# NIH-NEI/oct-image-segmentation-models

Measured on AMD Instinct MI355X. Metric: B-scans/sec (train step), 256x512 3-class U-Net, higher is better.
Workload: dtype f32; 1 GPU; configs[1]: train step (fwd+Dice-macro+bwd+allreduce+Adam), per-GPU batch 32, 256x512x1, 3-class, pool_layers=4, start_neurons=8, random-init weights; global_batch=32, parallelism=dp1, allreduce=none

## Files before the change

oct-image-segmentation-models_amd/csrc/common.hpp:

```cpp
#pragma once
#include <hip/hip_runtime.h>
#include <stdint.h>

namespace oct {

constexpr int kTileX = 32;
constexpr int kTileY = 8;
constexpr int kBlock = 256;

enum { BN_A = 0, BN_B = 1, BN_MEAN = 2, BN_RSTD = 3, BN_C1 = 4, BN_C2 = 5, BN_GA = 6, BN_GB = 7, BN_GD = 8, BN_ARRAYS = 9 };

enum { F_U8 = 1, F_AFF = 2, F_TWO = 4, F_UP = 8, F_DROP = 16 };

static __constant__ float c_u8_lut[256];

__host__ __device__ inline uint32_t drop_hash(uint64_t seed, uint64_t step, uint32_t idx) {
    uint64_t x = seed ^ (step * 0x9E3779B97F4A7C15ull) ^ ((uint64_t)idx * 0xD1B54A32D192ED03ull);
    x ^= x >> 33; x *= 0xff51afd7ed558ccdull;
    x ^= x >> 33; x *= 0xc4ceb9fe1a85ec53ull;
    x ^= x >> 33;
    return (uint32_t)(x >> 32);
}

struct DropCfg {
// ... 32 lines not shown
template <int N, bool WT = false>
__device__ inline void block_reduce_store(float (&v)[N], float* red, float* out, int nvalid) {
    wave_reduce_multi<N>(v);
    const int lane = threadIdx.x & 63, wave = threadIdx.x >> 6;
    red[wave * 64 + lane] = v[0];
    __syncthreads();
    if ((int)threadIdx.x < N && (int)threadIdx.x < nvalid) {
        const int l = threadIdx.x * (64 / N);
        const float r = (red[l] + red[64 + l]) + (red[128 + l] + red[192 + l]);
        if constexpr (WT) __hip_atomic_store(out + threadIdx.x, r, __ATOMIC_RELAXED, __HIP_MEMORY_SCOPE_AGENT);
        else out[threadIdx.x] = r;
    }
    __syncthreads();
}

template <int N>
__host__ __device__ inline int chan_of_lane(int lane) {
    int c = 0, n = N, off = 32;
    while (n > 1) { if (lane & off) c += n / 2; n >>= 1; off >>= 1; }
    return c;
}

__device__ inline void column_sums_f64(const float* __restrict__ part, int rows, int C, int c, double* sh, double& s, double& q) {
    s = 0; q = 0;
    const size_t ld = 2 * (size_t)C;
    int i = threadIdx.x;
    for (; i + 7 * kBlock < rows; i += 8 * kBlock) {
        float a[8], b[8];
#pragma unroll
        for (int k = 0; k < 8; ++k) { const float* r = part + (size_t)(i + k * kBlock) * ld + c; a[k] = r[0]; b[k] = r[C]; }
        s += (((double)a[0] + a[1]) + ((double)a[2] + a[3])) + (((double)a[4] + a[5]) + ((double)a[6] + a[7]));
        q += (((double)b[0] + b[1]) + ((double)b[2] + b[3])) + (((double)b[4] + b[5]) + ((double)b[6] + b[7]));
    }
    {
        float a[7], b[7];
#pragma unroll
        for (int k = 0; k < 7; ++k) {
            const int r_ = i + k * kBlock; const bool ok = r_ < rows;
            const float* r = part + (size_t)(ok ? r_ : 0) * ld + c;
            a[k] = ok ? r[0] : 0.f; b[k] = ok ? r[C] : 0.f;
        }
#pragma unroll
        for (int k = 0; k < 7; ++k) { s += a[k]; q += b[k]; }
    }
#pragma unroll
    for (int o = 32; o > 0; o >>= 1) { s += __shfl_xor(s, o, 64); q += __shfl_xor(q, o, 64); }
    const int wave = threadIdx.x >> 6;
    if ((threadIdx.x & 63) == 0) { sh[wave] = s; sh[4 + wave] = q; }
    __syncthreads();
    s = (sh[0] + sh[1]) + (sh[2] + sh[3]); q = (sh[4] + sh[5]) + (sh[6] + sh[7]);
}

__device__ inline float4 ld4(const float* p) { return *reinterpret_cast<const float4*>(p); }
__device__ inline void st4(float* p, const float4& v) { *reinterpret_cast<float4*>(p) = v; }

typedef unsigned short bf16_t;
__device__ inline float bf2f(bf16_t h) { return __uint_as_float(((uint32_t)h) << 16); }
__device__ inline bf16_t f2bf(float f) {
    const uint32_t u = __float_as_uint(f);
    return (bf16_t)((u + 0x7FFFu + ((u >> 16) & 1u)) >> 16);
}
template <typename AT> __device__ inline float4 lda4(const AT* p);
template <> __device__ inline float4 lda4<float>(const float* p) { return *reinterpret_cast<const float4*>(p); }
template <> __device__ inline float4 lda4<bf16_t>(const bf16_t* p) {
    const uint2 u = *reinterpret_cast<const uint2*>(p);
    return make_float4(__uint_as_float(u.x << 16), __uint_as_float(u.x & 0xFFFF0000u),
                       __uint_as_float(u.y << 16), __uint_as_float(u.y & 0xFFFF0000u));
}
template <typename AT> struct Raw4;
template <> struct Raw4<float> { using type = float4; };
template <> struct Raw4<bf16_t> { using type = uint2; };
template <typename AT> __device__ inline typename Raw4<AT>::type ldraw4(const AT* p);
template <> __device__ inline float4 ldraw4<float>(const float* p) { return *reinterpret_cast<const float4*>(p); }
template <> __device__ inline uint2 ldraw4<bf16_t>(const bf16_t* p) { return *reinterpret_cast<const uint2*>(p); }
template <typename AT> __device__ inline typename Raw4<AT>::type raw_zero4();
template <> __device__ inline float4 raw_zero4<float>() { return make_float4(0.f, 0.f, 0.f, 0.f); }
template <> __device__ inline uint2 raw_zero4<bf16_t>() { return make_uint2(0u, 0u); }
__device__ inline float4 widen4(const float4& r) { return r; }
__device__ inline float4 widen4(const uint2& u) {
    return make_float4(__uint_as_float(u.x << 16), __uint_as_float(u.x & 0xFFFF0000u),
                       __uint_as_float(u.y << 16), __uint_as_float(u.y & 0xFFFF0000u));
}
template <typename AT> __device__ inline void sta4(AT* p, const float4& v);
template <> __device__ inline void sta4<float>(float* p, const float4& v) { *reinterpret_cast<float4*>(p) = v; }
typedef __bf16 bf16x2_hw __attribute__((ext_vector_type(2)));
typedef float f32x2_hw __attribute__((ext_vector_type(2)));
template <> __device__ inline void sta4<bf16_t>(bf16_t* p, const float4& v) {
    uint2 u;
    u.x = __builtin_bit_cast(uint32_t, __builtin_convertvector(f32x2_hw{v.x, v.y}, bf16x2_hw));
    u.y = __builtin_bit_cast(uint32_t, __builtin_convertvector(f32x2_hw{v.z, v.w}, bf16x2_hw));
    *reinterpret_cast<uint2*>(p) = u;
}
template <typename AT> __device__ inline float lda1(const AT* p);
template <> __device__ inline float lda1<float>(const float* p) { return *p; }
template <> __device__ inline float lda1<bf16_t>(const bf16_t* p) { return bf2f(*p); }

}
```

oct-image-segmentation-models_amd/csrc/kernels_bwd.hpp:

```cpp
#pragma once
#include "common.hpp"
#include "kernels_fwd.hpp"

namespace oct {

struct PoolBwdArgs {
    const void* gp;
    const void* z;
    const float* bn;
    void* g;
    float* part;
    int H, W, C, tiles_x, tiles, act_bf16;
    FinDesc fin;
};

template <int C_T, typename AT>
__global__ __launch_bounds__(kBlock) void pool_bwd_k(const PoolBwdArgs A) {
    __shared__ float red[256];
    const int Ho = A.H >> 1, Wo = A.W >> 1;
    const int tx = threadIdx.x & (kTileX - 1), ty = threadIdx.x / kTileX;
    const int tile = blockIdx.x;
    const int xo = (tile % A.tiles_x) * kTileX + tx, yo = (tile / A.tiles_x) * kTileY + ty;
    const int b = blockIdx.z, c0 = blockIdx.y * C_T;
    const bool valid = xo < Wo && yo < Ho;
// ... 165 lines not shown
        const uint4 gr = *reinterpret_cast<const uint4*>(g + i * 8), zr = *reinterpret_cast<const uint4*>(z + i * 8);
        const float4 gv[2] = {widen4(make_uint2(gr.x, gr.y)), widen4(make_uint2(gr.z, gr.w))};
        const float4 zv[2] = {widen4(make_uint2(zr.x, zr.y)), widen4(make_uint2(zr.z, zr.w))};
        bf16_t* out = g + i * 8;
#pragma unroll
        for (int hlf = 0; hlf < 2; ++hlf) {
            const int cc = c + 4 * hlf;
            const float4 ga = ld4(bn + BN_GA * C + cc), gb = ld4(bn + BN_GB * C + cc), gd = ld4(bn + BN_GD * C + cc);
            float4 o;
            o.x = bn_bwd_apply1(ga.x, gb.x, gd.x, gv[hlf].x, zv[hlf].x);
            o.y = bn_bwd_apply1(ga.y, gb.y, gd.y, gv[hlf].y, zv[hlf].y);
            o.z = bn_bwd_apply1(ga.z, gb.z, gd.z, gv[hlf].z, zv[hlf].z);
            o.w = bn_bwd_apply1(ga.w, gb.w, gd.w, gv[hlf].w, zv[hlf].w);
            sta4<bf16_t>(out + 4 * hlf, o);
        }
    }
}

struct HeadBwdArgs {
    const void* z; const float* bn;
    const float* w; const float* bias;
    const unsigned char* labels;
    const double* bc;
    void* g;
    float* part;
    float* wpart;
    int HW, nblk, B, macro; float loss_scale; int act_bf16;
    float focal_w, focal_gamma; const float* focal_cw; float inv_count;
    int focal_clip_mod;
    int bce_on; float bce_inner, bce_scale;
    FinDesc fin;
};

template <int C, int CIN, typename AT>
__global__ __launch_bounds__(kBlock) void head_bwd_k(const HeadBwdArgs A) {
    constexpr int NV = CIN * C + C, NG = (NV + 31) / 32;
    constexpr int CP = CIN <= 4 ? 4 : (CIN <= 8 ? 8 : (CIN <= 16 ? 16 : 32));
    __shared__ float red[256];
    const int b = blockIdx.y;
    float s1[CP], s2[CP], wv[NG * 32];
#pragma unroll
    for (int i = 0; i < CP; ++i) { s1[i] = 0.f; s2[i] = 0.f; }
#pragma unroll
    for (int i = 0; i < NG * 32; ++i) wv[i] = 0.f;
    float num[C], den[C];
#pragma unroll
    for (int c = 0; c < C; ++c) {
        const double* k = A.macro ? A.bc + 2 * (b * C + c) : A.bc + 2 * A.B * C;
        num[c] = (float)k[0]; den[c] = (float)k[1];
    }
    const float scale = (1.f - A.focal_w) * (A.macro ? A.loss_scale / (float)(A.B * C) : A.loss_scale);
    const float fscale = A.focal_w * A.loss_scale * A.inv_count;

    const AT* const zbase = reinterpret_cast<const AT*>(A.z) + (size_t)b * A.HW * CIN;
    auto pix_of = [&](int chunk) { const int px = chunk * kBlock + threadIdx.x; return px < A.HW ? px : 0; };
    float zn[CIN];
    int labn = 0;
    if ((int)blockIdx.x * kBlock < A.HW) {
        const int q = pix_of(blockIdx.x);
        head_load<CIN, AT>(zbase + (size_t)q * CIN, zn);
        labn = A.labels[(size_t)b * A.HW + q];
    }
    for (int chunk = blockIdx.x; chunk * kBlock < A.HW; chunk += gridDim.x) {
        const int px = chunk * kBlock + threadIdx.x;
        const bool valid = px < A.HW;
        const size_t pix = (size_t)b * A.HW + (valid ? px : 0);
        float y[CIN], zr[CIN], p[C];
#pragma unroll
        for (int i = 0; i < CIN; ++i) zr[i] = zn[i];
        const int lab = labn;
        if ((chunk + (int)gridDim.x) * kBlock < A.HW) {
            const int q = pix_of(chunk + gridDim.x);
            head_load<CIN, AT>(zbase + (size_t)q * CIN, zn);
            labn = A.labels[(size_t)b * A.HW + q];
        }
        head_logits<C, CIN>(A.bn, A.w, A.bias, y, zr, p);
        float dp[C], dot = 0.f;
#pragma unroll
        for (int c = 0; c < C; ++c) {
            const float yv = lab == c ? 1.f : 0.f;
            dp[c] = -scale * (2.f * yv * den[c] - num[c]) / (den[c] * den[c]);
            if (fscale != 0.f && lab == c) {
                const bool inr = p[c] >= kFocalEps && p[c] <= 1.f - kFocalEps;
                if (inr || !A.focal_clip_mod) {
                    const float pc = fminf(fmaxf(p[c], kFocalEps), 1.f - kFocalEps);
                    const float q = 1.f - p[c], cw = A.focal_cw ? A.focal_cw[c] : 1.f, qg1 = powf(q, A.focal_gamma - 1.f);
                    dp[c] += fscale * cw * (A.focal_gamma * qg1 * logf(pc) - (inr ? qg1 * q / pc : 0.f));
                }
            }
            dot = fmaf(p[c], dp[c], dot);
        }
        float dlb[C];
#pragma unroll
        for (int c = 0; c < C; ++c) dlb[c] = 0.f;
        if (A.bce_on) {
            float q[C], db[C];
            softmax_complement<C>(p, q);
#pragma unroll
            for (int c = 0; c < C; ++c) {
                const bool inr = valid && p[c] >= kFocalEps && q[c] >= kFocalEps;
                const float r = A.bce_scale / ((lab == c ? p[c] : q[c]) + A.bce_inner);
                db[c] = inr ? (lab == c ? -r : r) : 0.f;
            }
#pragma unroll
            for (int c = 0; c < C; ++c) {
                float o = 0.f;
#pragma unroll
                for (int k = 0; k < C; ++k) if (k != c) o = fmaf(p[k], db[k], o);
                dlb[c] = p[c] * (q[c] * db[c] - o);
            }
        }
        float dl[C];
#pragma unroll
        for (int c = 0; c < C; ++c) { dl[c] = (valid ? p[c] * (dp[c] - dot) : 0.f) + dlb[c]; wv[CIN * C + c] += dl[c]; }
        float g[CIN];
#pragma unroll
        for (int i = 0; i < CIN; ++i) {
            float a = 0.f;
#pragma unroll
            for (int c = 0; c < C; ++c) { a = fmaf(A.w[i * C + c], dl[c], a); wv[i * C + c] = fmaf(y[i], dl[c], wv[i * C + c]); }
            a = (valid && y[i] > 0.f) ? a : 0.f;
            const float xh = (zr[i] - A.bn[BN_MEAN * CIN + i]) * A.bn[BN_RSTD * CIN + i];
            g[i] = a; s1[i] += a; s2[i] += a * xh;
        }
        if (valid) {
#pragma unroll
            for (int i = 0; i < CIN; i += 4) sta4<AT>(reinterpret_cast<AT*>(A.g) + pix * CIN + i, make_float4(g[i], g[i + 1], g[i + 2], g[i + 3]));
        }
    }
    const size_t row = (size_t)b * gridDim.x + blockIdx.x;
    float* out = A.part + row * (2 * CIN);
    block_reduce_store<CP, true>(s1, red, out, CIN);
    block_reduce_store<CP, true>(s2, red, out + CIN, CIN);
    float* wout = A.wpart + row * NV;
#pragma unroll
    for (int gi = 0; gi < NG; ++gi) {
        float t[32];
#pragma unroll
        for (int k = 0; k < 32; ++k) t[k] = wv[gi * 32 + k];
        block_reduce_store<32>(t, red, wout + gi * 32, NV - gi * 32 < 32 ? NV - gi * 32 : 32);
    }
    if (A.fin.counter) {
        __shared__ __attribute__((aligned(16))) char fin_lds[16 + kBlock * 16 + 2 * CP * 8];
        finalize_in_launch(A.fin, A.part, gridDim.x * gridDim.y, CIN, gridDim.x * gridDim.y, fin_lds);
    }
}

struct ConvBwdWArgs {
    const void* x0; const float* ab0; int C0;
    const void* x1; const float* ab1; int C1;
    int flags;
    const void* dz;
    const void* zf; const float* bnf;
    float* part;
    int B, H, W, Cin, Cout, tiles_x, tiles, total_tiles, npb;
    DropCfg drop;
    int act_bf16;
};

__device__ __forceinline__ float fetch_x(const ConvBwdWArgs& A, int b, int iy, int ix, int c) {
    const bool up = (A.flags & F_UP) != 0;
    const int Hs = up ? A.H >> 1 : A.H, Ws = up ? A.W >> 1 : A.W;
    const int sy = up ? iy >> 1 : iy, sx = up ? ix >> 1 : ix;
    const size_t pix = ((size_t)b * Hs + sy) * Ws + sx;
    if (A.flags & F_U8) return c_u8_lut[reinterpret_cast<const unsigned char*>(A.x0)[pix * A.C0 + c]];
    const float* src = reinterpret_cast<const float*>(A.x0); const float* ab = A.ab0; int C = A.C0, cc = c;
    if ((A.flags & F_TWO) && c >= A.C0) { src = reinterpret_cast<const float*>(A.x1); ab = A.ab1; C = A.C1; cc = c - A.C0; }
    float v = src[pix * C + cc];
    if (A.flags & F_AFF) v = fmaxf(fmaf(ab[cc], v, ab[C + cc]), 0.f);
    if (A.flags & F_DROP) v *= drop_mul(A.drop, (uint32_t)(pix * C + cc));
    return v;
}

template <int KH, int CI_T, int CO_T, typename AT>
__global__ __launch_bounds__(kBlock) void conv_bwd_w_k(const ConvBwdWArgs A) {
// ... 8 lines not shown
    float acc[TAPS], accb = 0.f;
#pragma unroll
    for (int k = 0; k < TAPS; ++k) acc[k] = 0.f;

    for (int tl = blockIdx.x; tl < A.total_tiles; tl += A.npb) {
        const int b = tl / A.tiles, tile = tl % A.tiles;
        const int x0 = (tile % A.tiles_x) * kTileX, y0 = (tile / A.tiles_x) * kTileY;
        __syncthreads();
        for (int i = t; i < XH * XW * CI_T; i += kBlock) {
            const int c = i % CI_T, r = i / CI_T, cx = r % XW, cy = r / XW;
            const int iy = y0 + cy - PT, ix = x0 + cx - PT;
            float v = 0.f;
            if (iy >= 0 && iy < A.H && ix >= 0 && ix < A.W && ci0 + c < A.Cin) v = fetch_x(A, b, iy, ix, ci0 + c);
            Xs[i] = v;
        }
        for (int i = t; i < kTileY * kTileX * CO_T; i += kBlock) {
            const int c = i % CO_T, r = i / CO_T, cx = r % kTileX, cy = r / kTileX;
            const int oy = y0 + cy, ox = x0 + cx;
            float v = 0.f;
            if (oy < A.H && ox < A.W && co0 + c < A.Cout) v = lda1<AT>(reinterpret_cast<const AT*>(A.dz) + (((size_t)b * A.H + oy) * A.W + ox) * A.Cout + co0 + c);
            Ds[i] = v;
        }
        __syncthreads();
        for (int p = ps; p < kTileY * kTileX; p += PS) {
            const int py = p / kTileX, pxx = p % kTileX;
            const float d = Ds[p * CO_T + co];
            accb += d;
#pragma unroll
            for (int ky = 0; ky < KH; ++ky)
#pragma unroll
                for (int kx = 0; kx < KW; ++kx)
                    acc[ky * KW + kx] = fmaf(Xs[((py + ky) * XW + pxx + kx) * CI_T + ci], d, acc[ky * KW + kx]);
        }
    }
#pragma unroll
    for (int k = 0; k < TAPS; ++k) Rs[t * (TAPS + 1) + k] = acc[k];
    Rs[t * (TAPS + 1) + TAPS] = accb;
    __syncthreads();
    if (t < NT) {
        const size_t wsize = (size_t)TAPS * A.Cin * A.Cout;
        float* out = A.part + (size_t)blockIdx.x * (wsize + A.Cout);
        const bool ok = (ci0 + ci < A.Cin) && (co0 + co < A.Cout);
        for (int k = 0; k <= TAPS; ++k) {
            float s = 0.f;
            for (int q = 0; q < PS; ++q) s += Rs[(q * NT + t) * (TAPS + 1) + k];
            if (!ok) continue;
            if (k < TAPS) out[((size_t)k * A.Cin + ci0 + ci) * A.Cout + co0 + co] = s;
            else if (ci0 + ci == 0) out[wsize + co0 + co] = s;
        }
    }
}

template <typename AT, bool FUSE>
__global__ __launch_bounds__(kBlock) void conv_dw_first_k(const ConvBwdWArgs A, int tiles_x, int tiles, int total_tiles) {
    constexpr int TH = 8, TW = 128, XH = TH + 2, XW = TW + 2;
    __shared__ float Xs[XH * XW];
    __shared__ float red[256];
    __shared__ float lut_s[256];
    const int t = threadIdx.x, xl = t & 31, row = t >> 5;
    lut_s[t] = c_u8_lut[t];
    float acc0[64], acc1[16];
#pragma unroll
    for (int k = 0; k < 64; ++k) acc0[k] = 0.f;
#pragma unroll
    for (int k = 0; k < 16; ++k) acc1[k] = 0.f;
    const bool u8 = (A.flags & F_U8) != 0;
    for (int tl = blockIdx.x; tl < total_tiles; tl += gridDim.x) {
        const int b = tl / tiles, tile = tl % tiles;
        const int x0 = (tile % tiles_x) * TW, y0 = (tile / tiles_x) * TH;
        __syncthreads();
        {
            constexpr int NS = (XH * XW + kBlock - 1) / kBlock;
            unsigned int rb[NS]; float rf[NS]; bool in[NS];
#pragma unroll
            for (int k = 0; k < NS; ++k) {
                const int i = t + k * kBlock, cy = i / XW, cx = i % XW, iy = y0 + cy - 1, ix = x0 + cx - 1;
                in[k] = i < XH * XW && iy >= 0 && iy < A.H && ix >= 0 && ix < A.W;
                const size_t pix = in[k] ? ((size_t)b * A.H + iy) * A.W + ix : 0;
                rb[k] = 0; rf[k] = 0.f;
                if (in[k]) { if (u8) rb[k] = reinterpret_cast<const unsigned char*>(A.x0)[pix]; else rf[k] = reinterpret_cast<const float*>(A.x0)[pix]; }
            }
#pragma unroll
            for (int k = 0; k < NS; ++k) {
                const int i = t + k * kBlock;
                if (i < XH * XW) Xs[i] = in[k] ? (u8 ? lut_s[rb[k]] : rf[k]) : 0.f;
            }
        }
        __syncthreads();
        const int y = y0 + row;
#pragma unroll
        for (int k = 0; k < TW / 32; ++k) {
            const int xx = xl + 32 * k, x = x0 + xx;
            if (y < A.H && x < A.W) {
                const size_t e8 = (((size_t)b * A.H + y) * A.W + x) * 8;
                const AT* dp = reinterpret_cast<const AT*>(A.dz) + e8;
                const float4 d0 = lda4<AT>(dp), d1 = lda4<AT>(dp + 4);
                float d[8] = {d0.x, d0.y, d0.z, d0.w, d1.x, d1.y, d1.z, d1.w};
                if constexpr (FUSE) {
                    const AT* zp = reinterpret_cast<const AT*>(A.zf) + e8;
                    const float4 z0 = lda4<AT>(zp), z1 = lda4<AT>(zp + 4);
                    const float zv[8] = {z0.x, z0.y, z0.z, z0.w, z1.x, z1.y, z1.z, z1.w};
#pragma unroll
                    for (int co = 0; co < 8; ++co) {
                        const float o = bn_bwd_apply1(A.bnf[BN_GA * 8 + co], A.bnf[BN_GB * 8 + co], A.bnf[BN_GD * 8 + co], d[co], zv[co]);
                        d[co] = dz_as_stored<AT>(o);
                        asm volatile("" : "+v"(d[co]));
                    }
                }
#pragma unroll
                for (int tap = 0; tap < 9; ++tap) {
                    const float xv = Xs[(row + tap / 3) * XW + xx + tap % 3];
#pragma unroll
                    for (int co = 0; co < 8; ++co) {
                        if (tap < 8) acc0[tap * 8 + co] = fmaf(xv, d[co], acc0[tap * 8 + co]);
                        else acc1[co] = fmaf(xv, d[co], acc1[co]);
                    }
                }
#pragma unroll
                for (int co = 0; co < 8; ++co) acc1[8 + co] += d[co];
            }
        }
    }
    float* out = A.part + (size_t)blockIdx.x * 80;
    block_reduce_store<64>(acc0, red, out, 64);
    block_reduce_store<16>(acc1, red, out + 64, 16);
}

template <int JW>
__global__ __launch_bounds__(kBlock) void reduce_partials_k(const float* __restrict__ part, int npb, size_t stride,
                                                           size_t wsize, float* __restrict__ dw, float* __restrict__ db) {
    constexpr int NQ = kBlock / JW;
    __shared__ double sh[NQ][JW];
    const int col = threadIdx.x % JW, q = threadIdx.x / JW;
    const size_t j = (size_t)blockIdx.x * JW + col;
    double s = 0;
    if (j < stride)
        for (int p = q; p < npb; p += NQ) s += part[(size_t)p * stride + j];
    sh[q][col] = s;
    __syncthreads();
    if (q == 0 && j < stride) {
        double t = 0;
#pragma unroll
        for (int k = 0; k < NQ; ++k) t += sh[k][col];
        if (j < wsize) dw[j] = (float)t; else db[j - wsize] = (float)t;
    }
}

struct ReduceAllArgs {
    static constexpr int MAXL = 40;
    int n;
    struct Entry { const float* part; float* dw; float* db; int npb, jw; unsigned stride, wsize, blk_start; } L[MAXL];
};

static __global__ __launch_bounds__(kBlock) void reduce_all_k(const ReduceAllArgs A) {
    __shared__ double sh[kBlock];
    int d = 0;
    while (d + 1 < A.n && blockIdx.x >= A.L[d + 1].blk_start) ++d;
    const ReduceAllArgs::Entry E = A.L[d];
    const int jw = E.jw, nq = kBlock / jw, col = threadIdx.x % jw, q = threadIdx.x / jw;
    const size_t j = (size_t)(blockIdx.x - E.blk_start) * jw + col;
    double s = 0;
    if (j < E.stride) {
        const float* __restrict__ src = E.part + j;
        int p = q;
        for (; p + 7 * nq < E.npb; p += 8 * nq) {
            float v[8];
#pragma unroll
            for (int k = 0; k < 8; ++k) v[k] = src[(size_t)(p + k * nq) * E.stride];
            s += (((double)v[0] + v[1]) + ((double)v[2] + v[3])) + (((double)v[4] + v[5]) + ((double)v[6] + v[7]));
        }
        for (; p < E.npb; p += nq) s += src[(size_t)p * E.stride];
    }
    sh[q * jw + col] = s;
    __syncthreads();
// ... 28 lines not shown
```

oct-image-segmentation-models_amd/csrc/kernels_fwd.hpp:

```cpp
#pragma once
#include "common.hpp"
#include "kernels_fin.hpp"

namespace oct {

struct ConvFwdArgs {
    const void* x0;
    const float* ab0;
    int C0;
    const float* x1;
    const float* ab1;
    int C1;
    const float* w;
    const float* bias;
    void* z;
    float* part;
    int H, W, Cin, Cout, tiles_x, tiles;
    DropCfg drop;
    int act_bf16;
    FinDesc fin;
};

template <int CO_T, int FLAGS>
__device__ inline void accum_src(const void* __restrict__ src, const float* __restrict__ ab, int C, size_t pix,
// ... 36 lines not shown
            if constexpr (U8) v = c_u8_lut[reinterpret_cast<const unsigned char*>(src)[pix * C + c]];
            else v = reinterpret_cast<const float*>(src)[pix * C + c];
            if constexpr (AFF) v = fmaxf(fmaf(ab[c], v, ab[C + c]), 0.f);
        }
        const float* wr = wk + (size_t)c * Cout;
#pragma unroll
        for (int j = 0; j < CO_T; ++j) acc[j] = fmaf(v, wr[j], acc[j]);
    }
}

template <int KH, int CO_T, int FLAGS, typename AT>
__global__ __launch_bounds__(kBlock) void conv_fwd_k(const ConvFwdArgs A) {
    constexpr int KW = KH, PT = (KH - 1) / 2;
    constexpr bool TWO = (FLAGS & F_TWO) != 0, UP = (FLAGS & F_UP) != 0;
    __shared__ float red[256];
    const int tx = threadIdx.x & (kTileX - 1), ty = threadIdx.x / kTileX;
    const int tile = blockIdx.x;
    const int x = (tile % A.tiles_x) * kTileX + tx, y = (tile / A.tiles_x) * kTileY + ty;
    const int b = blockIdx.z, co0 = blockIdx.y * CO_T;
    const bool valid = x < A.W && y < A.H;
    const int Hs = UP ? A.H >> 1 : A.H, Ws = UP ? A.W >> 1 : A.W;

    float acc[CO_T];
#pragma unroll
    for (int j = 0; j < CO_T; ++j) acc[j] = A.bias[co0 + j];

    for (int ky = 0; ky < KH; ++ky) {
        for (int kx = 0; kx < KW; ++kx) {
            const int iy = y + ky - PT, ix = x + kx - PT;
            const bool inb = valid && iy >= 0 && iy < A.H && ix >= 0 && ix < A.W;
            const int sy = UP ? iy >> 1 : iy, sx = UP ? ix >> 1 : ix;
            const size_t pix = inb ? ((size_t)b * Hs + sy) * Ws + sx : 0;
            const float* wk = A.w + (size_t)((ky * KW + kx) * A.Cin) * A.Cout + co0;
            accum_src<CO_T, FLAGS>(A.x0, A.ab0, A.C0, pix, inb, wk, A.Cout, A.drop, acc);
            if constexpr (TWO)
                accum_src<CO_T, FLAGS>(A.x1, A.ab1, A.C1, pix, inb, wk + (size_t)A.C0 * A.Cout, A.Cout, A.drop, acc);
        }
    }
    if (valid) {
        AT* zp = reinterpret_cast<AT*>(A.z) + (((size_t)b * A.H + y) * A.W + x) * A.Cout + co0;
#pragma unroll
        for (int j = 0; j < CO_T; j += 4) sta4<AT>(zp + j, make_float4(acc[j], acc[j + 1], acc[j + 2], acc[j + 3]));
    }
    if (A.part) {
        float s[CO_T], q[CO_T];
#pragma unroll
        for (int j = 0; j < CO_T; ++j) { s[j] = valid ? acc[j] : 0.f; q[j] = s[j] * s[j]; }
        float* out = A.part + ((size_t)b * A.tiles + tile) * (2 * A.Cout);
        block_reduce_store<CO_T>(s, red, out + co0, CO_T);
        block_reduce_store<CO_T>(q, red, out + A.Cout + co0, CO_T);
    }
}

template <typename AT>
__global__ __launch_bounds__(kBlock) void conv_first_fwd_k(const ConvFwdArgs A, int x_is_u8, int tiles_x, int tiles, int total_tiles,
                                                          const float* __restrict__ wgt, const float* __restrict__ bias) {
    constexpr int TH = 8, TW = 128, XH = TH + 2, XW = TW + 2;
    __shared__ float Xs[XH * XW];
    __shared__ float red[256];
    __shared__ float lut_s[256];
    const int t = threadIdx.x, xl = t & 31, row = t >> 5;
    lut_s[t] = c_u8_lut[t];
    float s1[8], s2[8];
#pragma unroll
    for (int j = 0; j < 8; ++j) { s1[j] = 0.f; s2[j] = 0.f; }
    for (int tl = blockIdx.x; tl < total_tiles; tl += gridDim.x) {
        const int b = tl / tiles, tile = tl % tiles;
        const int x0 = (tile % tiles_x) * TW, y0 = (tile / tiles_x) * TH;
        __syncthreads();
        {
            constexpr int NS = (XH * XW + kBlock - 1) / kBlock;
            unsigned int rb[NS]; float rf[NS]; bool in[NS];
#pragma unroll
            for (int k = 0; k < NS; ++k) {
                const int i = t + k * kBlock, cy = i / XW, cx = i % XW, iy = y0 + cy - 1, ix = x0 + cx - 1;
                in[k] = i < XH * XW && iy >= 0 && iy < A.H && ix >= 0 && ix < A.W;
                const size_t pix = in[k] ? ((size_t)b * A.H + iy) * A.W + ix : 0;
                rb[k] = 0; rf[k] = 0.f;
                if (in[k]) { if (x_is_u8) rb[k] = reinterpret_cast<const unsigned char*>(A.x0)[pix]; else rf[k] = reinterpret_cast<const float*>(A.x0)[pix]; }
            }
#pragma unroll
            for (int k = 0; k < NS; ++k) {
                const int i = t + k * kBlock;
                if (i < XH * XW) Xs[i] = in[k] ? (x_is_u8 ? lut_s[rb[k]] : rf[k]) : 0.f;
            }
        }
        __syncthreads();
        const int y = y0 + row;
#pragma unroll
        for (int k = 0; k < TW / 32; ++k) {
            const int xx = xl + 32 * k, x = x0 + xx;
            float acc[8];
#pragma unroll
            for (int j = 0; j < 8; ++j) acc[j] = bias[j];
#pragma unroll
            for (int tap = 0; tap < 9; ++tap) {
                const float xv = Xs[(row + tap / 3) * XW + xx + tap % 3];
#pragma unroll
                for (int j = 0; j < 8; ++j) acc[j] = fmaf(xv, wgt[tap * 8 + j], acc[j]);
            }
            if (y < A.H && x < A.W) {
                AT* zp = reinterpret_cast<AT*>(A.z) + (((size_t)b * A.H + y) * A.W + x) * 8;
                sta4<AT>(zp, make_float4(acc[0], acc[1], acc[2], acc[3]));
                sta4<AT>(zp + 4, make_float4(acc[4], acc[5], acc[6], acc[7]));
#pragma unroll
                for (int j = 0; j < 8; ++j) { s1[j] += acc[j]; s2[j] = fmaf(acc[j], acc[j], s2[j]); }
// ... 64 lines not shown
        const int c = (int)(i % C4) * 4;
        size_t r = i / C4;
        const int xo = (int)(r % Wo); r /= Wo;
        const int yo = (int)(r % Ho); const int b = (int)(r / Ho);
        const float4 a = ld4(ab + c), bb = ld4(ab + C + c);
        float4 m = make_float4(0.f, 0.f, 0.f, 0.f);
#pragma unroll
        for (int dy = 0; dy < 2; ++dy)
#pragma unroll
            for (int dx = 0; dx < 2; ++dx) {
                const float4 v = lda4<AT>(z + (((size_t)b * H + 2 * yo + dy) * W + 2 * xo + dx) * C + c);
                m.x = fmaxf(m.x, fmaf(a.x, v.x, bb.x)); m.y = fmaxf(m.y, fmaf(a.y, v.y, bb.y));
                m.z = fmaxf(m.z, fmaf(a.z, v.z, bb.z)); m.w = fmaxf(m.w, fmaf(a.w, v.w, bb.w));
            }
        sta4<AT>(p + (((size_t)b * Ho + yo) * Wo + xo) * C + c, m);
    }
}

constexpr int kDiceVals = 5;
template <int C> struct DiceN { static constexpr int value = (5 * C <= 16) ? 16 : (5 * C <= 32 ? 32 : 64); };

struct HeadFwdArgs {
    const void* z; const float* ab;
    const float* w; const float* bias;
    float* probs; unsigned char* argmax; const unsigned char* labels;
    float* dice_part;
    int HW, nblk, act_bf16;
    int focal_on; float focal_gamma; const float* focal_cw;
    int focal_clip_mod;
    int bce_on; float bce_inner;
};
constexpr float kFocalEps = 1e-7f;

template <int C>
__device__ inline void softmax_complement(const float (&p)[C], float (&q)[C]) {
#pragma unroll
    for (int c = 0; c < C; ++c) {
        float s = 0.f;
#pragma unroll
        for (int k = 0; k < C; ++k) if (k != c) s += p[k];
        q[c] = s;
    }
}

template <int CIN, typename AT>
__device__ inline void head_load(const AT* __restrict__ zp, float (&zr)[CIN]) {
#pragma unroll
    for (int i = 0; i < CIN; i += 4) {
        const float4 v = lda4<AT>(zp + i);
        zr[i] = v.x; zr[i + 1] = v.y; zr[i + 2] = v.z; zr[i + 3] = v.w;
    }
}

template <int C, int CIN>
__device__ inline void head_logits(const float* __restrict__ ab, const float* __restrict__ w, const float* __restrict__ bias,
                                   float (&y)[CIN], const float (&zr)[CIN], float (&p)[C]) {
#pragma unroll
    for (int i = 0; i < CIN; ++i) y[i] = fmaxf(fmaf(ab[i], zr[i], ab[CIN + i]), 0.f);
    float mx = -3.4e38f;
#pragma unroll
    for (int c = 0; c < C; ++c) {
        float l = bias[c];
#pragma unroll
        for (int i = 0; i < CIN; ++i) l = fmaf(y[i], w[i * C + c], l);
        p[c] = l; mx = fmaxf(mx, l);
    }
    float sum = 0.f;
#pragma unroll
    for (int c = 0; c < C; ++c) { p[c] = expf(p[c] - mx); sum += p[c]; }
    const float inv = 1.f / sum;
#pragma unroll
    for (int c = 0; c < C; ++c) p[c] *= inv;
}

template <int C, int CIN, typename AT>
__global__ __launch_bounds__(kBlock) void head_fwd_k(const HeadFwdArgs A) {
    constexpr int N = DiceN<C>::value;
    __shared__ float red[256];
    const int b = blockIdx.y;
    float v[N];
#pragma unroll
    for (int i = 0; i < N; ++i) v[i] = 0.f;
    for (int chunk = blockIdx.x; chunk * kBlock < A.HW; chunk += gridDim.x) {
        const int px = chunk * kBlock + threadIdx.x;
        const bool valid = px < A.HW;
        const size_t pix = (size_t)b * A.HW + (valid ? px : 0);
        float y[CIN], zr[CIN], p[C];
        head_load<CIN, AT>(reinterpret_cast<const AT*>(A.z) + pix * CIN, zr);
        head_logits<C, CIN>(A.ab, A.w, A.bias, y, zr, p);
        if (valid) {
            if (A.probs) {
#pragma unroll
                for (int c = 0; c < C; ++c) A.probs[pix * C + c] = p[c];
            }
            if (A.argmax) {
                int am = 0; float best = p[0];
#pragma unroll
                for (int c = 1; c < C; ++c) if (p[c] > best) { best = p[c]; am = c; }
                A.argmax[pix] = (unsigned char)am;
            }
            if (A.labels) {
                const int lab = A.labels[pix];
#pragma unroll
                for (int c = 0; c < C; ++c) {
                    const float yv = lab == c ? 1.f : 0.f, ph = p[c] > 0.5f ? 1.f : 0.f;
                    v[c * kDiceVals + 0] += yv * p[c]; v[c * kDiceVals + 1] += yv; v[c * kDiceVals + 2] += p[c];
                    v[c * kDiceVals + 3] += yv * ph;   v[c * kDiceVals + 4] += ph;
                }
                if (A.focal_on) {
                    float py = p[0];
#pragma unroll
                    for (int c = 1; c < C; ++c) py = lab == c ? p[c] : py;
                    const float pc = fminf(fmaxf(py, kFocalEps), 1.f - kFocalEps);
                    const float cw = A.focal_cw ? A.focal_cw[lab < C ? lab : 0] : 1.f;
                    v[C * kDiceVals] += cw * powf(1.f - (A.focal_clip_mod ? pc : py), A.focal_gamma) * -logf(pc);
                }
                if (A.bce_on) {
                    float q[C], t = 0.f;
                    softmax_complement<C>(p, q);
#pragma unroll
                    for (int c = 0; c < C; ++c) {
                        const float u = lab == c ? p[c] : q[c];
                        t -= logf(fminf(fmaxf(u, kFocalEps), 1.f - kFocalEps) + A.bce_inner);
                    }
                    v[C * kDiceVals] += t;
                }
            }
        }
    }
    if (A.labels) block_reduce_store<N>(v, red, A.dice_part + ((size_t)b * gridDim.x + blockIdx.x) * N, N);
}

struct DiceFinArgs {
    const float* part; int B, C, nblk, N;
    float smooth; float* out4; float* out4_user; double* bc;
    int n_user;
    double inv_count;
    float focal_w;
    int bce_on;
};

static __global__ __launch_bounds__(kBlock) void dice_finalize_k(const DiceFinArgs A) {
    __shared__ double sh[8][kBlock];
    double acc[8] = {0, 0, 0, 0, 0, 0, 0, 0};
    const int n = A.B * A.C;
    for (int i = threadIdx.x; i < n; i += kBlock) {
        const int b = i / A.C, c = i % A.C;
        double v[kDiceVals] = {0, 0, 0, 0, 0};
        const float* p0 = A.part + (size_t)b * A.nblk * A.N + c * kDiceVals;
        int k = 0;
        for (; k + 8 <= A.nblk; k += 8) {
            float t[8][kDiceVals];
#pragma unroll
            for (int r = 0; r < 8; ++r)
#pragma unroll
                for (int j = 0; j < kDiceVals; ++j) t[r][j] = p0[(size_t)(k + r) * A.N + j];
#pragma unroll
            for (int r = 0; r < 8; ++r)
#pragma unroll
                for (int j = 0; j < kDiceVals; ++j) v[j] += t[r][j];
        }
        for (; k < A.nblk; ++k)
            for (int j = 0; j < kDiceVals; ++j) v[j] += p0[(size_t)k * A.N + j];
        const double s = A.smooth;
        const double num = 2.0 * v[0] + s, den = v[1] + v[2] + s;
        A.bc[2 * i] = num; A.bc[2 * i + 1] = den;
        acc[0] += num / den;
        acc[1] += (2.0 * v[3] + 1e-5) / (v[1] + v[4] + 1e-5);
        acc[2] += v[0]; acc[3] += v[1]; acc[4] += v[2]; acc[5] += v[3]; acc[6] += v[4];
        if (c == 0)
            for (int k = 0; k < A.nblk; ++k) acc[7] += A.part[((size_t)b * A.nblk + k) * A.N + A.C * kDiceVals];
    }
    for (int j = 0; j < 8; ++j) sh[j][threadIdx.x] = acc[j];
    __syncthreads();
    for (int o = kBlock / 2; o > 0; o >>= 1) {
        if ((int)threadIdx.x < o) for (int j = 0; j < 8; ++j) sh[j][threadIdx.x] += sh[j][threadIdx.x + o];
        __syncthreads();
    }
    if (threadIdx.x == 0) {
        const double s = A.smooth;
        const double num = 2.0 * sh[2][0] + s, den = sh[3][0] + sh[4][0] + s;
        A.bc[2 * n] = num; A.bc[2 * n + 1] = den;
        float o4[8];
        o4[0] = (float)(1.0 - sh[0][0] / n);
        o4[1] = (float)(1.0 - num / den);
        o4[2] = (float)(sh[1][0] / n);
        o4[3] = (float)(2.0 * sh[5][0] / (sh[3][0] + sh[6][0]));
        const double focal = sh[7][0] * A.inv_count, w = A.focal_w;
        o4[4] = (float)focal;
        o4[5] = (float)(w * focal + (1.0 - w) * (1.0 - sh[0][0] / n));
        o4[6] = (float)(w * focal + (1.0 - w) * (1.0 - num / den));
        o4[7] = 0.f;
        if (A.bce_on) {
            const double bce = sh[7][0] * (A.inv_count / A.C);
            o4[4] = (float)bce; o4[5] = 0.f; o4[6] = (float)(bce + (1.0 - num / den));
        }
        for (int j = 0; j < 8; ++j) { A.out4[j] = o4[j]; if (A.out4_user && j < A.n_user) A.out4_user[j] = o4[j]; }
    }
}

static __global__ __launch_bounds__(kBlock) void boundary_maps_k(const unsigned char* __restrict__ lab, unsigned char* __restrict__ out,
                                                         int B, int H, int W, int C, int bg_ilm, int bg_csi) {
    const size_t n = (size_t)B * H * W;
    for (size_t i = (size_t)blockIdx.x * kBlock + threadIdx.x; i < n; i += (size_t)gridDim.x * kBlock) {
        const int c = (int)(i % W); size_t t = i / W;
        const int r = (int)(t % H), b = (int)(t / H);
        const unsigned char* col = lab + (size_t)b * H * W + c;
        auto L = [&](int rr) { return (int)col[(size_t)rr * W]; };
        const int r1 = r + 1 == H ? 0 : r + 1;
        int lv[6];
        const int rows[6] = {r > 0 ? r - 1 : 0, r, r + 1 < H ? r + 1 : H - 1, r1 > 0 ? r1 - 1 : 0, r1, r1 + 1 < H ? r1 + 1 : H - 1};
#pragma unroll
        for (int k = 0; k < 6; ++k) lv[k] = L(rows[k]);
        for (int m = 1; m < C; ++m) {
            const bool flip = (m == 1 && bg_ilm) || (m == C - 1 && bg_csi);
            const int k = flip ? m - 1 : m;
            auto grad2 = [&](int rr, int lo, int mid, int hi) {
                int d2;
                if (H == 1) d2 = 0;
                else if (rr == 0) d2 = 2 * ((hi == k) - (mid == k));
                else if (rr == H - 1) d2 = 2 * ((mid == k) - (lo == k));
                else d2 = (hi == k) - (lo == k);
                if (flip) d2 = -d2;
                return d2 > 0 ? d2 : 0;
            };
            const int g0 = grad2(r, lv[0], lv[1], lv[2]);
// ... 14 lines not shown
```

Measured before the change: 8456 B-scans/s.

## Prefetch head and first-conv tiles, use constant-space loads, parallelize dice finalize

Adds a HeadQueue prefetcher to the forward and backward head kernels so the next chunk's activations and labels load while the current chunk is computed. conv_dw_first_k gets a double-buffered shared input tile with register staging, prefetches dz/zf loads two groups ahead, and raises occupancy via launch_bounds. Small parameter loads now go through the constant address space so they can use scalar loads. dice_finalize uses a deeper unrolled reduction and gives the focal-term sums to otherwise idle threads. These changes aim to hide memory latency, at the cost of more registers and shared memory.

```diff
diff --git a/oct-image-segmentation-models_amd/csrc/common.hpp b/oct-image-segmentation-models_amd/csrc/common.hpp
--- a/oct-image-segmentation-models_amd/csrc/common.hpp
+++ b/oct-image-segmentation-models_amd/csrc/common.hpp
@@ -108,6 +108,7 @@
 }
 
 __device__ inline float4 ld4(const float* p) { return *reinterpret_cast<const float4*>(p); }
+__device__ __forceinline__ float ldc(const float* p) { return *(const __attribute__((address_space(4))) float*)p; }
 __device__ inline void st4(float* p, const float4& v) { *reinterpret_cast<float4*>(p) = v; }
 
 typedef unsigned short bf16_t;
diff --git a/oct-image-segmentation-models_amd/csrc/kernels_bwd.hpp b/oct-image-segmentation-models_amd/csrc/kernels_bwd.hpp
--- a/oct-image-segmentation-models_amd/csrc/kernels_bwd.hpp
+++ b/oct-image-segmentation-models_amd/csrc/kernels_bwd.hpp
@@ -241,28 +241,14 @@
     const float scale = (1.f - A.focal_w) * (A.macro ? A.loss_scale / (float)(A.B * C) : A.loss_scale);
     const float fscale = A.focal_w * A.loss_scale * A.inv_count;
 
-    const AT* const zbase = reinterpret_cast<const AT*>(A.z) + (size_t)b * A.HW * CIN;
-    auto pix_of = [&](int chunk) { const int px = chunk * kBlock + threadIdx.x; return px < A.HW ? px : 0; };
-    float zn[CIN];
-    int labn = 0;
-    if ((int)blockIdx.x * kBlock < A.HW) {
-        const int q = pix_of(blockIdx.x);
-        head_load<CIN, AT>(zbase + (size_t)q * CIN, zn);
-        labn = A.labels[(size_t)b * A.HW + q];
-    }
+    HeadQueue<CIN, kHeadBwdAhead, AT> hq(reinterpret_cast<const AT*>(A.z) + (size_t)b * A.HW * CIN, A.labels + (size_t)b * A.HW, A.HW);
+    hq.fill(blockIdx.x, gridDim.x);
     for (int chunk = blockIdx.x; chunk * kBlock < A.HW; chunk += gridDim.x) {
         const int px = chunk * kBlock + threadIdx.x;
         const bool valid = px < A.HW;
         const size_t pix = (size_t)b * A.HW + (valid ? px : 0);
         float y[CIN], zr[CIN], p[C];
-#pragma unroll
-        for (int i = 0; i < CIN; ++i) zr[i] = zn[i];
-        const int lab = labn;
-        if ((chunk + (int)gridDim.x) * kBlock < A.HW) {
-            const int q = pix_of(chunk + gridDim.x);
-            head_load<CIN, AT>(zbase + (size_t)q * CIN, zn);
-            labn = A.labels[(size_t)b * A.HW + q];
-        }
+        const int lab = hq.pop(zr, chunk + kHeadBwdAhead * (int)gridDim.x);
         head_logits<C, CIN>(A.bn, A.w, A.bias, y, zr, p);
         float dp[C], dot = 0.f;
 #pragma unroll
@@ -273,7 +259,7 @@
                 const bool inr = p[c] >= kFocalEps && p[c] <= 1.f - kFocalEps;
                 if (inr || !A.focal_clip_mod) {
                     const float pc = fminf(fmaxf(p[c], kFocalEps), 1.f - kFocalEps);
-                    const float q = 1.f - p[c], cw = A.focal_cw ? A.focal_cw[c] : 1.f, qg1 = powf(q, A.focal_gamma - 1.f);
+                    const float q = 1.f - p[c], cw = A.focal_cw ? ldc(A.focal_cw + c) : 1.f, qg1 = powf(q, A.focal_gamma - 1.f);
                     dp[c] += fscale * cw * (A.focal_gamma * qg1 * logf(pc) - (inr ? qg1 * q / pc : 0.f));
                 }
             }
@@ -307,9 +293,9 @@
         for (int i = 0; i < CIN; ++i) {
             float a = 0.f;
 #pragma unroll
-            for (int c = 0; c < C; ++c) { a = fmaf(A.w[i * C + c], dl[c], a); wv[i * C + c] = fmaf(y[i], dl[c], wv[i * C + c]); }
+            for (int c = 0; c < C; ++c) { a = fmaf(ldc(A.w + i * C + c), dl[c], a); wv[i * C + c] = fmaf(y[i], dl[c], wv[i * C + c]); }
             a = (valid && y[i] > 0.f) ? a : 0.f;
-            const float xh = (zr[i] - A.bn[BN_MEAN * CIN + i]) * A.bn[BN_RSTD * CIN + i];
+            const float xh = (zr[i] - ldc(A.bn + BN_MEAN * CIN + i)) * ldc(A.bn + BN_RSTD * CIN + i);
             g[i] = a; s1[i] += a; s2[i] += a * xh;
         }
         if (valid) {
@@ -424,9 +410,9 @@
 }
 
 template <typename AT, bool FUSE>
-__global__ __launch_bounds__(kBlock) void conv_dw_first_k(const ConvBwdWArgs A, int tiles_x, int tiles, int total_tiles) {
-    constexpr int TH = 8, TW = 128, XH = TH + 2, XW = TW + 2;
-    __shared__ float Xs[XH * XW];
+__global__ __launch_bounds__(kBlock, 3) void conv_dw_first_k(const ConvBwdWArgs A, int tiles_x, int tiles, int total_tiles) {
+    constexpr int TH = FirstTileRaw::TH, TW = FirstTileRaw::TW, XH = FirstTileRaw::XH, XW = FirstTileRaw::XW, NG = TW / 32;
+    __shared__ float Xs2[2][XH * XW];
     __shared__ float red[256];
     __shared__ float lut_s[256];
     const int t = threadIdx.x, xl = t & 31, row = t >> 5;
@@ -437,44 +423,47 @@
 #pragma unroll
     for (int k = 0; k < 16; ++k) acc1[k] = 0.f;
     const bool u8 = (A.flags & F_U8) != 0;
-    for (int tl = blockIdx.x; tl < total_tiles; tl += gridDim.x) {
+    FirstTileRaw nx;
+    const bool any = (int)blockIdx.x < total_tiles;
+    if (any) nx.request(A.x0, u8, blockIdx.x, tiles, tiles_x, A.H, A.W);
+    __syncthreads();
+    if (any) nx.store(Xs2[0], lut_s, u8);
+    __syncthreads();
+    int cur = 0;
+    for (int tl = blockIdx.x; tl < total_tiles; tl += gridDim.x, cur ^= 1) {
         const int b = tl / tiles, tile = tl % tiles;
         const int x0 = (tile % tiles_x) * TW, y0 = (tile / tiles_x) * TH;
-        __syncthreads();
-        {
-            constexpr int NS = (XH * XW + kBlock - 1) / kBlock;
-            unsigned int rb[NS]; float rf[NS]; bool in[NS];
-#pragma unroll
-            for (int k = 0; k < NS; ++k) {
-                const int i = t + k * kBlock, cy = i / XW, cx = i % XW, iy = y0 + cy - 1, ix = x0 + cx - 1;
-                in[k] = i < XH * XW && iy >= 0 && iy < A.H && ix >= 0 && ix < A.W;
-                const size_t pix = in[k] ? ((size_t)b * A.H + iy) * A.W + ix : 0;
-                rb[k] = 0; rf[k] = 0.f;
-                if (in[k]) { if (u8) rb[k] = reinterpret_cast<const unsigned char*>(A.x0)[pix]; else rf[k] = reinterpret_cast<const float*>(A.x0)[pix]; }
-            }
-#pragma unroll
-            for (int k = 0; k < NS; ++k) {
-                const int i = t + k * kBlock;
-                if (i < XH * XW) Xs[i] = in[k] ? (u8 ? lut_s[rb[k]] : rf[k]) : 0.f;
-            }
-        }
-        __syncthreads();
+        const float* __restrict__ Xs = Xs2[cur];
+        const bool more = tl + (int)gridDim.x < total_tiles;
+        if (more) nx.request(A.x0, u8, tl + gridDim.x, tiles, tiles_x, A.H, A.W);
         const int y = y0 + row;
-#pragma unroll
-        for (int k = 0; k < TW / 32; ++k) {
-            const int xx = xl + 32 * k, x = x0 + xx;
-            if (y < A.H && x < A.W) {
-                const size_t e8 = (((size_t)b * A.H + y) * A.W + x) * 8;
-                const AT* dp = reinterpret_cast<const AT*>(A.dz) + e8;
-                const float4 d0 = lda4<AT>(dp), d1 = lda4<AT>(dp + 4);
-                float d[8] = {d0.x, d0.y, d0.z, d0.w, d1.x, d1.y, d1.z, d1.w};
+        constexpr int AH = 2;
+        float4 dq[NG][2]; [[maybe_unused]] float4 zq[NG][2];
+        bool ok[NG];
+        auto request = [&](int k) {
+            const int x = x0 + xl + 32 * k;
+            ok[k] = y < A.H && x < A.W;
+            const size_t e8 = ok[k] ? (((size_t)b * A.H + y) * A.W + x) * 8 : 0;
+            const AT* dp = reinterpret_cast<const AT*>(A.dz) + e8;
+            dq[k][0] = lda4<AT>(dp); dq[k][1] = lda4<AT>(dp + 4);
+            if constexpr (FUSE) {
+                const AT* zp = reinterpret_cast<const AT*>(A.zf) + e8;
+                zq[k][0] = lda4<AT>(zp); zq[k][1] = lda4<AT>(zp + 4);
+            }
+        };
+#pragma unroll
+        for (int k = 0; k < AH; ++k) request(k);
+#pragma unroll
+        for (int k = 0; k < NG; ++k) {
+            if (k + AH < NG) request(k + AH);
+            const int xx = xl + 32 * k;
+            if (ok[k]) {
+                float d[8] = {dq[k][0].x, dq[k][0].y, dq[k][0].z, dq[k][0].w, dq[k][1].x, dq[k][1].y, dq[k][1].z, dq[k][1].w};
                 if constexpr (FUSE) {
-                    const AT* zp = reinterpret_cast<const AT*>(A.zf) + e8;
-                    const float4 z0 = lda4<AT>(zp), z1 = lda4<AT>(zp + 4);
-                    const float zv[8] = {z0.x, z0.y, z0.z, z0.w, z1.x, z1.y, z1.z, z1.w};
+                    const float zv[8] = {zq[k][0].x, zq[k][0].y, zq[k][0].z, zq[k][0].w, zq[k][1].x, zq[k][1].y, zq[k][1].z, zq[k][1].w};
 #pragma unroll
                     for (int co = 0; co < 8; ++co) {
-                        const float o = bn_bwd_apply1(A.bnf[BN_GA * 8 + co], A.bnf[BN_GB * 8 + co], A.bnf[BN_GD * 8 + co], d[co], zv[co]);
+                        const float o = bn_bwd_apply1(ldc(A.bnf + BN_GA * 8 + co), ldc(A.bnf + BN_GB * 8 + co), ldc(A.bnf + BN_GD * 8 + co), d[co], zv[co]);
                         d[co] = dz_as_stored<AT>(o);
                         asm volatile("" : "+v"(d[co]));
                     }
@@ -492,6 +481,8 @@
                 for (int co = 0; co < 8; ++co) acc1[8 + co] += d[co];
             }
         }
+        if (more) nx.store(Xs2[cur ^ 1], lut_s, u8);
+        __syncthreads();
     }
     float* out = A.part + (size_t)blockIdx.x * 80;
     block_reduce_store<64>(acc0, red, out, 64);
diff --git a/oct-image-segmentation-models_amd/csrc/kernels_fwd.hpp b/oct-image-segmentation-models_amd/csrc/kernels_fwd.hpp
--- a/oct-image-segmentation-models_amd/csrc/kernels_fwd.hpp
+++ b/oct-image-segmentation-models_amd/csrc/kernels_fwd.hpp
@@ -112,6 +112,34 @@
     }
 }
 
+struct FirstTileRaw {
+    static constexpr int TH = 8, TW = 128, XH = TH + 2, XW = TW + 2, NS = (XH * XW + kBlock - 1) / kBlock;
+    unsigned int raw[NS];
+    unsigned int inm;
+    __device__ __forceinline__ void request(const void* __restrict__ x, bool u8, int tl, int tiles, int tiles_x, int H, int W) {
+        const int b = tl / tiles, tile = tl % tiles, x0 = (tile % tiles_x) * TW, y0 = (tile / tiles_x) * TH;
+        inm = 0;
+#pragma unroll
+        for (int k = 0; k < NS; ++k) {
+            const int i = (int)threadIdx.x + k * kBlock, cy = i / XW, cx = i % XW, iy = y0 + cy - 1, ix = x0 + cx - 1;
+            const bool in = i < XH * XW && iy >= 0 && iy < H && ix >= 0 && ix < W;
+            const size_t pix = in ? ((size_t)b * H + iy) * W + ix : 0;
+            raw[k] = 0;
+            if (in) {
+                if (u8) raw[k] = reinterpret_cast<const unsigned char*>(x)[pix]; else raw[k] = __float_as_uint(reinterpret_cast<const float*>(x)[pix]);
+                inm |= 1u << k;
+            }
+        }
+    }
+    __device__ __forceinline__ void store(float* __restrict__ Xs, const float* __restrict__ lut_s, bool u8) const {
+#pragma unroll
+        for (int k = 0; k < NS; ++k) {
+            const int i = (int)threadIdx.x + k * kBlock;
+            if (i < XH * XW) Xs[i] = (inm >> k & 1u) ? (u8 ? lut_s[raw[k]] : __uint_as_float(raw[k])) : 0.f;
+        }
+    }
+};
+
 template <typename AT>
 __global__ __launch_bounds__(kBlock) void conv_first_fwd_k(const ConvFwdArgs A, int x_is_u8, int tiles_x, int tiles, int total_tiles,
                                                           const float* __restrict__ wgt, const float* __restrict__ bias) {
@@ -282,17 +310,49 @@
     }
 }
 
+constexpr int kHeadFwdAhead = 1, kHeadBwdAhead = 1;
+template <int CIN, int D, typename AT>
+struct HeadQueue {
+    const AT* zb; const unsigned char* lb; int HW;
+    float zq[D][CIN]; int lq[D];
+    __device__ HeadQueue(const AT* z, const unsigned char* l, int hw) : zb(z), lb(l), HW(hw) {}
+    __device__ __forceinline__ void request(int d, int chunk) {
+        if (chunk * kBlock < HW) {
+            const int px = chunk * kBlock + (int)threadIdx.x, q = px < HW ? px : 0;
+            head_load<CIN, AT>(zb + (size_t)q * CIN, zq[d]);
+            if (lb) lq[d] = lb[q];
+        }
+    }
+    __device__ __forceinline__ void fill(int first, int stride) {
+#pragma unroll
+        for (int d = 0; d < D; ++d) { lq[d] = 0; request(d, first + d * stride); }
+    }
+    __device__ __forceinline__ int pop(float (&zr)[CIN], int next) {
+        const int lab = lq[0];
+#pragma unroll
+        for (int i = 0; i < CIN; ++i) zr[i] = zq[0][i];
+#pragma unroll
+        for (int d = 0; d + 1 < D; ++d) {
+            lq[d] = lq[d + 1];
+#pragma unroll
+            for (int i = 0; i < CIN; ++i) zq[d][i] = zq[d + 1][i];
+        }
+        request(D - 1, next);
+        return lab;
+    }
+};
+
 template <int C, int CIN>
 __device__ inline void head_logits(const float* __restrict__ ab, const float* __restrict__ w, const float* __restrict__ bias,
                                    float (&y)[CIN], const float (&zr)[CIN], float (&p)[C]) {
 #pragma unroll
-    for (int i = 0; i < CIN; ++i) y[i] = fmaxf(fmaf(ab[i], zr[i], ab[CIN + i]), 0.f);
+    for (int i = 0; i < CIN; ++i) y[i] = fmaxf(fmaf(ldc(ab + i), zr[i], ldc(ab + CIN + i)), 0.f);
     float mx = -3.4e38f;
 #pragma unroll
     for (int c = 0; c < C; ++c) {
-        float l = bias[c];
-#pragma unroll
-        for (int i = 0; i < CIN; ++i) l = fmaf(y[i], w[i * C + c], l);
+        float l = ldc(bias + c);
+#pragma unroll
+        for (int i = 0; i < CIN; ++i) l = fmaf(y[i], ldc(w + i * C + c), l);
         p[c] = l; mx = fmaxf(mx, l);
     }
     float sum = 0.f;
@@ -311,12 +371,15 @@
     float v[N];
 #pragma unroll
     for (int i = 0; i < N; ++i) v[i] = 0.f;
+    HeadQueue<CIN, kHeadFwdAhead, AT> hq(reinterpret_cast<const AT*>(A.z) + (size_t)b * A.HW * CIN,
+                                         A.labels ? A.labels + (size_t)b * A.HW : nullptr, A.HW);
+    hq.fill(blockIdx.x, gridDim.x);
     for (int chunk = blockIdx.x; chunk * kBlock < A.HW; chunk += gridDim.x) {
         const int px = chunk * kBlock + threadIdx.x;
         const bool valid = px < A.HW;
         const size_t pix = (size_t)b * A.HW + (valid ? px : 0);
         float y[CIN], zr[CIN], p[C];
-        head_load<CIN, AT>(reinterpret_cast<const AT*>(A.z) + pix * CIN, zr);
+        const int lab = hq.pop(zr, chunk + kHeadFwdAhead * (int)gridDim.x);
         head_logits<C, CIN>(A.ab, A.w, A.bias, y, zr, p);
         if (valid) {
             if (A.probs) {
@@ -330,7 +393,6 @@
                 A.argmax[pix] = (unsigned char)am;
             }
             if (A.labels) {
-                const int lab = A.labels[pix];
 #pragma unroll
                 for (int c = 0; c < C; ++c) {
                     const float yv = lab == c ? 1.f : 0.f, ph = p[c] > 0.5f ? 1.f : 0.f;
@@ -370,38 +432,56 @@
     int bce_on;
 };
 
+template <int R, int J>
+__device__ __forceinline__ int dice_rows(const float* __restrict__ p0, int N, int k, int nblk, double (&v)[J]) {
+    for (; k + R <= nblk; k += R) {
+        float t[R][J];
+#pragma unroll
+        for (int r = 0; r < R; ++r)
+#pragma unroll
+            for (int j = 0; j < J; ++j) t[r][j] = p0[(size_t)(k + r) * N + j];
+#pragma unroll
+        for (int r = 0; r < R; ++r)
+#pragma unroll
+            for (int j = 0; j < J; ++j) v[j] += t[r][j];
+    }
+    return k;
+}
+template <int J>
+__device__ __forceinline__ void dice_rows_all(const float* __restrict__ p0, int N, int nblk, double (&v)[J]) {
+    int k = dice_rows<32, J>(p0, N, 0, nblk, v);
+    k = dice_rows<8, J>(p0, N, k, nblk, v);
+    dice_rows<1, J>(p0, N, k, nblk, v);
+}
+
 static __global__ __launch_bounds__(kBlock) void dice_finalize_k(const DiceFinArgs A) {
     __shared__ double sh[8][kBlock];
     double acc[8] = {0, 0, 0, 0, 0, 0, 0, 0};
     const int n = A.B * A.C;
+    const int hb = kBlock - 1 - (int)threadIdx.x;
+    const bool helper = hb < A.B && n + hb < kBlock;
+    double hs[1] = {0};
+    if (helper) dice_rows_all<1>(A.part + (size_t)hb * A.nblk * A.N + A.C * kDiceVals, A.N, A.nblk, hs);
     for (int i = threadIdx.x; i < n; i += kBlock) {
         const int b = i / A.C, c = i % A.C;
         double v[kDiceVals] = {0, 0, 0, 0, 0};
         const float* p0 = A.part + (size_t)b * A.nblk * A.N + c * kDiceVals;
-        int k = 0;
-        for (; k + 8 <= A.nblk; k += 8) {
-            float t[8][kDiceVals];
-#pragma unroll
-            for (int r = 0; r < 8; ++r)
-#pragma unroll
-                for (int j = 0; j < kDiceVals; ++j) t[r][j] = p0[(size_t)(k + r) * A.N + j];
-#pragma unroll
-            for (int r = 0; r < 8; ++r)
-#pragma unroll
-                for (int j = 0; j < kDiceVals; ++j) v[j] += t[r][j];
-        }
-        for (; k < A.nblk; ++k)
-            for (int j = 0; j < kDiceVals; ++j) v[j] += p0[(size_t)k * A.N + j];
+        dice_rows_all<kDiceVals>(p0, A.N, A.nblk, v);
         const double s = A.smooth;
         const double num = 2.0 * v[0] + s, den = v[1] + v[2] + s;
         A.bc[2 * i] = num; A.bc[2 * i + 1] = den;
         acc[0] += num / den;
         acc[1] += (2.0 * v[3] + 1e-5) / (v[1] + v[4] + 1e-5);
         acc[2] += v[0]; acc[3] += v[1]; acc[4] += v[2]; acc[5] += v[3]; acc[6] += v[4];
-        if (c == 0)
-            for (int k = 0; k < A.nblk; ++k) acc[7] += A.part[((size_t)b * A.nblk + k) * A.N + A.C * kDiceVals];
+        if (c == 0 && n + b >= kBlock) {
+            double f[1] = {acc[7]};
+            dice_rows_all<1>(A.part + (size_t)b * A.nblk * A.N + A.C * kDiceVals, A.N, A.nblk, f);
+            acc[7] = f[0];
+        }
     }
     for (int j = 0; j < 8; ++j) sh[j][threadIdx.x] = acc[j];
+    __syncthreads();
+    if (helper) sh[7][hb * A.C] = hs[0];
     __syncthreads();
     for (int o = kBlock / 2; o > 0; o >>= 1) {
         if ((int)threadIdx.x < o) for (int j = 0; j < 8; ++j) sh[j][threadIdx.x] += sh[j][threadIdx.x + o];
```

New measurement: 8579 B-scans/s, median of 6. 1.5% higher.
